# baiwenjia/ukbb_cardiac

Measured on AMD Instinct MI355X. Metric: 192x208 SAX slices/sec, higher is better.
Workload: dtype f32; 1 GPU; short-axis FCN (FCN_sa, 4 classes) inference, batch=64 synthetic 192x208 slices per GPU resident in HBM, int32 label map out (BASELINE.json configs[1]); height=192, width=208, weights=synthetic seed 1234, parallelism=batch split x1, no collectives

## Files before the change

### include/ukbb_fcn.h

```cpp
#ifndef UKBB_FCN_H
#define UKBB_FCN_H

#include <stddef.h>
#include <stdint.h>

#ifdef __cplusplus
extern "C" {
#endif

#define UKBB_FCN_ABI_VERSION 11
#define UKBB_FCN_MAX_LEVEL 8

#define UKBB_OK 0
#define UKBB_EINVAL (-1)
#define UKBB_EARCH (-2)
#define UKBB_EDEVICE (-3)
#define UKBB_ENOMEM (-4)

#define UKBB_KIND_FCN 0
#define UKBB_KIND_UNET 1
#define UKBB_KIND_UNET_LSTM 2
#define UKBB_KIND_TEMPORAL_UNET 3

typedef struct ukbb_fcn_arch {
// ... 79 lines not shown
                           int64_t st, double mu, double den, int X2, int Y2, int x_pre, int y_pre, float *d_batch, void *stream);


int ukbb_fcn_label_components(const uint8_t *d_lab, int X, int Y, int Z, int T, int n_class, int min_size, int32_t *d_work,
                              int32_t *d_n_large, void *stream);

int ukbb_fcn_label_max(const void *d_vol, int nifti_datatype, int X, int Y, int Z, int T, int64_t sx, int64_t sy, int64_t sz, int64_t st,
                       const uint8_t *d_lab, int n_class, double *d_max, void *stream);

int ukbb_fcn_label_compact(const void *d_vol, int nifti_datatype, int X, int Y, int Z, int64_t sx, int64_t sy, int64_t sz, const uint8_t *d_lab,
                           int label, void *d_out, uint64_t *n_host, void *stream);

uint64_t ukbb_fcn_gzip_labels_bound(uint64_t n_voxels, int nifti_datatype, uint64_t prefix_len);
int64_t ukbb_fcn_gzip_labels(const uint8_t *labels, uint64_t n_voxels, int nifti_datatype, const uint8_t *prefix, uint64_t prefix_len,
                             uint8_t *out, uint64_t out_cap);
#define UKBB_GZIP_FIXED 0
#define UKBB_GZIP_DYNAMIC 1
int64_t ukbb_fcn_gzip_labels_mode(const uint8_t *labels, uint64_t n_voxels, int nifti_datatype, const uint8_t *prefix, uint64_t prefix_len,
                                  uint8_t *out, uint64_t out_cap, int mode);

int64_t ukbb_fcn_gunzip(const uint8_t *src, uint64_t src_len, uint8_t *dst, uint64_t dst_cap, int verify_crc);
uint32_t ukbb_fcn_gzip_crc(uint32_t crc, const uint8_t *data, uint64_t n);


int ukbb_fcn_num_kernels(const ukbb_fcn_handle *h);
const char *ukbb_fcn_kernel_name(const ukbb_fcn_handle *h, int i);
double ukbb_fcn_kernel_macs(const ukbb_fcn_handle *h, int i);
double ukbb_fcn_kernel_mfma_macs(const ukbb_fcn_handle *h, int i);
double ukbb_fcn_kernel_mfma_macs_issued(const ukbb_fcn_handle *h, int i);

int ukbb_fcn_kernel_config(const ukbb_fcn_handle *h, int i);
const char *ukbb_fcn_conv_config_name(int id);

int ukbb_fcn_set_timing(ukbb_fcn_handle *h, int enable);
int ukbb_fcn_set_timing_kernel(ukbb_fcn_handle *h, int kernel);
int ukbb_fcn_kernel_times(ukbb_fcn_handle *h, double *sum_ms, int64_t *count, int n, int reset);

int64_t ukbb_fcn_get_activation(ukbb_fcn_handle *h, const char *name, float *dst, int64_t cap);

int ukbb_fcn_clock_probe(int device, void *stream, int spin_us, double *mhz);

int ukbb_fcn_synth_volume(uint64_t seed, size_t n, float *d_out, void *stream);

#ifdef __cplusplus
}
#endif
#endif
```

### ukbb_cardiac_amd/_lib.py

```python
import ctypes as C
import os

import numpy as np

_HERE = os.path.dirname(os.path.abspath(__file__))
LIB_PATH = os.environ.get('UKBB_FCN_LIB') or os.path.join(_HERE, 'libukbb_fcn.so')
ABI_VERSION = 11
MAX_LEVEL = 8

EXPORTS = [
    'ukbb_fcn_abi_version', 'ukbb_fcn_last_error', 'ukbb_fcn_weight_count', 'ukbb_fcn_create',
    'ukbb_fcn_destroy', 'ukbb_fcn_reserve', 'ukbb_fcn_forward', 'ukbb_fcn_forward_host',
    'ukbb_fcn_num_kernels', 'ukbb_fcn_kernel_name', 'ukbb_fcn_kernel_macs', 'ukbb_fcn_set_timing',
    'ukbb_fcn_kernel_times', 'ukbb_fcn_get_activation', 'ukbb_fcn_kernel_config', 'ukbb_fcn_conv_config_name',
    'ukbb_fcn_set_timing_kernel', 'ukbb_fcn_set_precision', 'ukbb_fcn_kernel_mfma_macs',
    'ukbb_fcn_select_kth', 'ukbb_fcn_rescale_pack', 'ukbb_fcn_unpack_labels',
    'ukbb_fcn_roi_compact', 'ukbb_fcn_pairwise_sum', 'ukbb_fcn_zscore_pack',
    'ukbb_fcn_gzip_labels_bound', 'ukbb_fcn_gzip_labels', 'ukbb_fcn_gzip_labels_mode', 'ukbb_fcn_gunzip', 'ukbb_fcn_gzip_crc',
    'ukbb_fcn_forward_seq', 'ukbb_fcn_forward_cine', 'ukbb_fcn_clock_probe', 'ukbb_fcn_kernel_mfma_macs_issued',
    'ukbb_fcn_synth_volume',
    'ukbb_fcn_select_kth_t', 'ukbb_fcn_rescale_pack_t', 'ukbb_fcn_roi_compact_t', 'ukbb_fcn_pairwise_sum_t', 'ukbb_fcn_zscore_pack_t',
    'ukbb_fcn_label_components', 'ukbb_fcn_label_max', 'ukbb_fcn_label_compact',
    'ukbb_fcn_set_scratch_budget', 'ukbb_fcn_scratch_bytes', 'ukbb_fcn_cine_scratch_bytes',
    'ukbb_fcn_cine_min_scratch_bytes', 'ukbb_fcn_cine_chunk_windows',
]


class ArchStruct(C.Structure):
    _fields_ = [('kind', C.c_int32), ('n_class', C.c_int32), ('n_level', C.c_int32),
                ('n_filter', C.c_int32 * MAX_LEVEL), ('n_block', C.c_int32 * MAX_LEVEL),
                ('same_dim', C.c_int32), ('fc', C.c_int32)]


def arch_struct(arch) -> ArchStruct:
    s = ArchStruct()
    s.kind, s.n_class, s.n_level = arch.kind, arch.n_class, arch.n_level
    for i in range(arch.n_level):
        s.n_filter[i] = arch.n_filter[i]
        s.n_block[i] = arch.n_block[i]
    s.same_dim, s.fc = arch.same_dim, arch.fc
    return s


def _load():
    if not os.path.exists(LIB_PATH):
        raise ImportError(
            'ukbb_cardiac_amd: %s is missing. Build the gfx950 HIP library first '
# ... 118 lines not shown
```

### ukbb_cardiac_amd/csrc/engine.cpp

```cpp
#include "../../include/ukbb_fcn.h"
#include "kernels.h"

#include <algorithm>
#include <cmath>
#include <cstdarg>
#include <cstdio>
#include <cstdlib>
#include <cstring>
#include <map>
#include <memory>
#include <string>
#include <vector>

using namespace ukbb;

extern "C" int ukbb_fcn_debug_poison_lds(uint32_t pattern, void *stream);
extern "C" int ukbb_fcn_debug_fence_kernel(void *stream);

namespace {

thread_local std::string g_err;

void set_err(const char *fmt, ...) {
    char buf[1024];
// ... 2024 lines not shown

double ukbb_fcn_kernel_mfma_macs(const ukbb_fcn_handle *h, int i) {
    if (!h || i < 0 || i >= (int)h->ops.size()) return 0.0;
    const Op &op = h->ops[i];
    return (op.mfma_macs_per_image >= 0 ? op.mfma_macs_per_image : op.macs_per_image) * h->last_n;
}

double ukbb_fcn_kernel_mfma_macs_issued(const ukbb_fcn_handle *h, int i) {
    if (!h || i < 0 || i >= (int)h->ops.size()) return 0.0;
    const Op &op = h->ops[i];
    if (op.padded_macs_per_image >= 0) return op.padded_macs_per_image * h->last_n;
    return ukbb_fcn_kernel_mfma_macs(h, i);
}

int ukbb_fcn_set_precision(ukbb_fcn_handle *h, int precision) {
    if (!h || (precision != UKBB_PREC_FP32 && precision != UKBB_PREC_BF16 && precision != UKBB_PREC_F32X3)) { set_err("set_precision: bad argument"); return UKBB_EINVAL; }
    if (h->arch.kind == UKBB_KIND_TEMPORAL_UNET && precision == UKBB_PREC_BF16) {
        set_err("set_precision: the Temporal-UNet's 3-D convolutions are built for fp32 only (no bf16 plan)");
        return UKBB_EARCH;
    }
    if (precision != h->precision) {
        if (hipSetDevice(h->device) != hipSuccess || hipDeviceSynchronize() != hipSuccess) { set_err("set_precision: device sync failed"); return UKBB_EDEVICE; }
        h->precision = precision;
        h->plan_h = h->plan_w = 0;
    }
    return UKBB_OK;
}

int ukbb_fcn_kernel_config(const ukbb_fcn_handle *h, int i) {
    if (!h || i < 0 || i >= (int)h->ops.size() || (h->ops[i].kind != OP_CONV && h->ops[i].kind != OP_TCONV)) return -1;
    return h->ops[i].cfg;
}

const char *ukbb_fcn_conv_config_name(int id) {
    for (int i = 0; i < num_conv_configs(); ++i)
        if (conv_config(i).id == id) return conv_config(i).name;
    return "";
}

int ukbb_fcn_set_timing(ukbb_fcn_handle *h, int enable) {
    if (!h) { set_err("set_timing: NULL handle"); return UKBB_EINVAL; }
    int rc = collect_events(h);
    if (rc) return rc;
    h->timing = enable != 0;
    h->timing_only = -1;
    return UKBB_OK;
}

int ukbb_fcn_set_timing_kernel(ukbb_fcn_handle *h, int kernel) {
    if (!h) { set_err("set_timing_kernel: NULL handle"); return UKBB_EINVAL; }
    int rc = collect_events(h);
    if (rc) return rc;
    if (kernel >= (int)h->ops.size()) { set_err("set_timing_kernel: index out of range"); return UKBB_EINVAL; }
    h->timing = true;
    h->timing_only = kernel < 0 ? -1 : kernel;
    return UKBB_OK;
}

int ukbb_fcn_kernel_times(ukbb_fcn_handle *h, double *sum_ms, int64_t *count, int n, int reset) {
    if (!h) { set_err("kernel_times: NULL handle"); return UKBB_EINVAL; }
    int rc = collect_events(h);
    if (rc) return rc;
    const int m = std::min<int>(n, (int)h->ops.size());
    for (int i = 0; i < m; ++i) {
        if (sum_ms) sum_ms[i] = h->t_sum[i];
        if (count) count[i] = h->t_cnt[i];
// ... 56 lines not shown
```

### ukbb_cardiac_amd/csrc/kernels.h

```cpp
#pragma once
#include <hip/hip_runtime.h>
#include <stdint.h>

#include "device_state.h"

namespace ukbb {

inline int current_device() { int d = 0; return hipGetDevice(&d) == hipSuccess ? d : -1; }
inline int device_cu_count() {
    static PerDeviceInt cu;
    const int d = current_device();
    return cu.get(d, [d] { hipDeviceProp_t p; return d >= 0 && hipGetDeviceProperties(&p, d) == hipSuccess ? p.multiProcessorCount : 0; }, 256);
}
inline hipError_t allow_dynamic_lds(OncePerDevice &once, const void *kernel, int bytes) {
    return (hipError_t)once.run(current_device(), [&] {
        return (int)hipFuncSetAttribute(kernel, hipFuncAttributeMaxDynamicSharedMemorySize, bytes); });
}

template <int NCLS>
__device__ __forceinline__ int softmax_argmax(const float (&lg)[NCLS], float *p) {
    int best = 0; float m = lg[0];
#pragma unroll
    for (int c = 1; c < NCLS; ++c) if (lg[c] > m) { m = lg[c]; best = c; }
    bool near = false;
// ... 120 lines not shown
    const float *x;
    const float *w_s;
    const float *b_s;
    const float *w_g;
    float *out;
    long long npix;
    int cin;
};
hipError_t launch_sqg(const SqgArgs &a, hipStream_t s);
struct SqgMultiArgs { SqgArgs lv[4]; int nb[4]; };
hipError_t launch_sqg_multi(const SqgArgs lv[4], hipStream_t s);

struct HeadArgs {
    const float *conv0;
    const float *G[4];
    const float *w_s0;
    const float *b_s0;
    const float *w_o0;
    const float *b_o0;
    const float *w_o1;
    const float *b_o1;
    const float *w_o0x3;
    const float *w_o1x3;
    const float *w_lg;
    const float *b_lg;
    float *logits;
    float *prob;
    int32_t *pred;
    int N, H, W, n_class;
    int x3;
    int diag;
};
hipError_t launch_head(const HeadArgs &a, hipStream_t s);
void pack_sq(const float *w , int cin, float *dst );
void pack_rowmap_32x64(const float *w , int ld, float *dst );
void pack_head_lg(const float *w , int n_class, float *dst );
void pack_head_x3(const float *w , int k_in , float *dst );

void tconv_as_conv2x2(const float *w, int cin, int cout, float *dst);

struct TailArgs {
    const float *in0, *in1;
    const float *wA0, *wA1;
    const float *b0, *b1;
    const float *lg_w, *lg_b;
    float *logits, *prob;
    int32_t *pred;
    int N, H, W, ncls;
    unsigned long long *stamps;
    int seg_tiles;
};
hipError_t launch_unet_tail(const TailArgs &a, hipStream_t s);
void pack_tail_weights(const float *w0 , const float *w1 , float *dst0 , float *dst1 );

struct StemArgs {
    const float *image;
    const float *wA0, *wA1;
    const float *b0, *b1;
    float *out;
    int N, H, W;
};
hipError_t launch_unet_stem(const StemArgs &a, hipStream_t s);
void pack_stem_weights(const float *w0 , float *dst0 );

struct LogitsArgs {
    const float *in;
// ... 91 lines not shown
```

### ukbb_cardiac_amd/csrc/kernels_head.hip

```cpp
#include "kernels.h"

#include <cstdio>

#include <cstdlib>
#include <cstring>
#include <type_traits>

namespace ukbb {

typedef float f32x16 __attribute__((ext_vector_type(16)));
typedef float f32x4 __attribute__((ext_vector_type(4)));

__host__ __device__ __forceinline__ constexpr int rowmap(int r, int g) {
    return (r & 3) + 8 * (r >> 2) + 4 * g;
}

typedef float f32x2 __attribute__((ext_vector_type(2)));
typedef unsigned u32x4 __attribute__((ext_vector_type(4)));
#ifdef UKBB_NO_PACKED_F32
__device__ __forceinline__ float s_fma(float a, float b, float c) { float r; asm("v_fma_f32 %0, %1, %2, %3" : "=v"(r) : "v"(a), "v"(b), "v"(c)); return r; }
__device__ __forceinline__ f32x2 pk_fma(f32x2 a, f32x2 b, f32x2 c) { return f32x2{s_fma(a[0], b[0], c[0]), s_fma(a[1], b[1], c[1])}; }
#else
__device__ __forceinline__ f32x2 pk_fma(f32x2 a, f32x2 b, f32x2 c) {
    f32x2 r; asm("v_pk_fma_f32 %0, %1, %2, %3" : "=v"(r) : "v"(a), "v"(b), "v"(c)); return r;
}
#endif
#define MFMA32(a, b, c) __builtin_amdgcn_mfma_f32_32x32x2f32((a), (b), (c), 0, 0, 0)

__device__ __forceinline__ f32x4 ldg4(const float *p) { return *reinterpret_cast<const f32x4 *>(p); }

__device__ __forceinline__ f32x16 bias_tile(const float *bias, int g) {
    f32x16 acc;
#pragma unroll
    for (int j = 0; j < 4; ++j) {
// ... 345 lines not shown
            float s = 0.f;
#pragma unroll
            for (int j = 0; j < 4; ++j) {
                const f32x4 w = ldg4(wp + 4 * j);
#pragma unroll
                for (int i = 0; i < 4; ++i) s = fmaf(w[i], Q0[4 * j + i], s);
            }
#pragma unroll
            for (int j = 0; j < 4; ++j) {
                const f32x4 w = ldg4(wp + 16 + 4 * j);
#pragma unroll
                for (int i = 0; i < 4; ++i) s = fmaf(w[i], Q1[4 * j + i], s);
            }
            const float other = __shfl_xor(s, 32);
            lg[c] = (g == 0 ? s + other : other + s) + a.b_lg[c];
        }
        if (g == 0) {
            if (a.logits) {
#pragma unroll
                for (int c = 0; c < NCLS; ++c) a.logits[q * NCLS + c] = lg[c];
            }
            float pr[NCLS];
            const int best = softmax_argmax_opt<NCLS>(lg, a.prob != nullptr, pr);
            if (a.pred) a.pred[q] = best;
            if (a.prob) {
#pragma unroll
                for (int c = 0; c < NCLS; ++c) a.prob[q * NCLS + c] = pr[c];
            }
        }
    }
}

#ifdef UKBB_DIAG
__device__ unsigned long long g_hstamps[8];
#endif
constexpr int PX_WAVE = 8 * 64 * 4;
constexpr int L_GW = 0;
constexpr int L_PX = L_GW + 2 * GPIX * GSTRIDE;
template <bool X3> struct HeadLds {
    static constexpr int WS0 = L_PX + 4 * PX_WAVE;
    static constexpr int WO0 = WS0 + 512;
    static constexpr int WO1 = WO0 + (X3 ? 3072 : 2048);
    static constexpr int BS0 = WO1 + (X3 ? 6144 : 4096);
    static constexpr int BO0 = BS0 + 32;
    static constexpr int BO1 = BO0 + 64;
    static constexpr int WLG = BO1 + 64;
    static constexpr int BLG = WLG + 384;
    static constexpr int FLOATS = BLG + 8;
};
constexpr int HEADPC_LDS_FLOATS = HeadLds<false>::FLOATS;
constexpr int HEADPC_X3_LDS_FLOATS = HeadLds<true>::FLOATS;
static_assert(HEADPC_X3_LDS_FLOATS * 4 <= 160 * 1024, "head kernel LDS");

__device__ __forceinline__ f32x4 lds4(const float *p) { return *reinterpret_cast<const f32x4 *>(p); }

template <int N, int I = 0, class F>
__device__ __forceinline__ void unroll_n(F &&f) {
    if constexpr (I < N) { f(std::integral_constant<int, I>{}); unroll_n<N, I + 1>(f); }
}

__device__ __forceinline__ f32x16 bias_tile_lds(const float *bias, int g) {
    f32x16 acc;
#pragma unroll
    for (int j = 0; j < 4; ++j) {
        const f32x4 b = lds4(bias + 8 * j + 4 * g);
#pragma unroll
        for (int i = 0; i < 4; ++i) acc[4 * j + i] = b[i];
    }
    return acc;
}

__device__ __forceinline__ void chain_32to64_lds(const float *wp, int lane, const f32x16 &X, f32x16 &D0, f32x16 &D1) {
#pragma unroll
    for (int q4 = 0; q4 < 4; ++q4) {
        const f32x4 wa = lds4(wp + ((0 * 4 + q4) * 64 + lane) * 4);
        const f32x4 wb = lds4(wp + ((1 * 4 + q4) * 64 + lane) * 4);
#pragma unroll
        for (int i = 0; i < 4; ++i) {
            D0 = MFMA32(wa[i], X[4 * q4 + i], D0);
            D1 = MFMA32(wb[i], X[4 * q4 + i], D1);
        }
    }
}

typedef __bf16 hbf16x8 __attribute__((ext_vector_type(8)));
__device__ __forceinline__ unsigned pk_bf16(float lo, float hi) {
    const __bf16 l = (__bf16)lo, h = (__bf16)hi;
    return (unsigned)__builtin_bit_cast(unsigned short, l) | ((unsigned)__builtin_bit_cast(unsigned short, h) << 16);
}
__device__ __forceinline__ void split_pair(float x0, float x1, unsigned &h, unsigned &m, unsigned &l) {
    h = pk_bf16(x0, x1);
    const float r0 = x0 - __builtin_bit_cast(float, h << 16), r1 = x1 - __builtin_bit_cast(float, h & 0xffff0000u);
    m = pk_bf16(r0, r1);
    const float q0 = r0 - __builtin_bit_cast(float, m << 16), q1 = r1 - __builtin_bit_cast(float, m & 0xffff0000u);
    l = pk_bf16(q0, q1);
}
__device__ __forceinline__ f32x16 mfma_b16(const u32x4 &a, const u32x4 &b, const f32x16 &c) {
    return __builtin_amdgcn_mfma_f32_32x32x16_bf16(__builtin_bit_cast(hbf16x8, a), __builtin_bit_cast(hbf16x8, b), c, 0, 0, 0);
}

__host__ __device__ constexpr int sep_pb(int l) { return ((1 << l) - 1) >> 1; }
__host__ __device__ constexpr int sep_row0(int r0, int l) { return (r0 + sep_pb(l)) >> l; }
__host__ __device__ constexpr bool sep_row_used(int r0, int l, int k) {
    const int f = 1 << l, i = sep_row0(r0, l) + k;
    bool used = false;
    for (int t = 0; t < 4; ++t) {
        const int y = r0 + t + sep_pb(l);
        if ((y >> l) + 1 == i || ((y >> l) == i && (y & (f - 1)) != f - 1)) used = true;
    }
    return used;
}

template <int NCLS, bool X3 = false, bool DG = false>
__global__ __launch_bounds__(768) void fcn_head_pc_kernel(const HeadArgs a) {
    extern __shared__ __attribute__((aligned(16))) float lds[];
    using LM = HeadLds<X3>;
    constexpr int L_WS0 = LM::WS0, L_WO0 = LM::WO0, L_WO1 = LM::WO1, L_BS0 = LM::BS0, L_BO0 = LM::BO0, L_BO1 = LM::BO1, L_WLG = LM::WLG, L_BLG = LM::BLG;
    float *gw = lds + L_GW;
    float *px = lds + L_PX;
    const int tiles_x = a.W / HT, tiles_y = a.H / HT;
    const int ntiles = a.N * tiles_y * tiles_x;
    const int my_tiles = (ntiles - (int)blockIdx.x + (int)gridDim.x - 1) / (int)gridDim.x;
    const int nstages = 2 * my_tiles;
    const bool producer = __builtin_amdgcn_readfirstlane(threadIdx.x) >= 256;
    const int lane = threadIdx.x & 63, p = lane & 31, g = lane >> 5;

    {
        const int t = threadIdx.x;
        auto copy = [&](int dst, const float *src, int nfloat) {
            for (int i = t; i < nfloat; i += 768) lds[dst + i] = src[i];
        };
        copy(L_WS0, a.w_s0, 512);
        if constexpr (X3) { copy(L_WO0, a.w_o0x3, 3072); copy(L_WO1, a.w_o1x3, 6144); }
        else              { copy(L_WO0, a.w_o0, 2048);   copy(L_WO1, a.w_o1, 4096); }
        copy(L_BS0, a.b_s0, 32);  copy(L_BO0, a.b_o0, 64);   copy(L_BO1, a.b_o1, 64);
        copy(L_WLG, a.w_lg, 2 * NCLS * 32); copy(L_BLG, a.b_lg, NCLS);
    }

    if (producer) {
        const int tid = threadIdx.x - 256, pw = (tid >> 6) & 3, half = tid >> 8;
        constexpr int NIT = 7;
        u32x4 gv[NIT];
        const int sp32 = tid >> 4, c4 = tid & 15;
#ifndef UKBB_HEAD_RECOMPUTE_WINDOW_CONSTS
#define UKBB_HEAD_RECOMPUTE_WINDOW_CONSTS 0
#endif
// ... 164 lines not shown
        };
        if (my_tiles > 0) { g_load(0); g_store(0); }
        if (my_tiles > 1) { g_load(1); g_store(1); }
        __syncthreads();
        auto stage = [&](auto parc, auto bufc, auto rgc, int s) {
            constexpr int PAR = decltype(parc)::value, BUF = decltype(bufc)::value;
            if constexpr (DG) {
                gather(parc, bufc);
                hand_over();
            } else {
                gather_sep(parc, bufc, rgc);
                hand_over_sep(rgc);
            }
            __syncthreads();
            __syncthreads();
            if constexpr (PAR == 1) {
                const int k = s >> 1;
                if (k + 2 < my_tiles) { g_load(k + 2); g_store(BUF); }
            }
        };
        constexpr std::integral_constant<int, 0> I0{};
        constexpr std::integral_constant<int, 1> I1{};
        auto run = [&](auto rgc) {
#pragma unroll 1
            for (int s = 0; s < nstages; s += 4) {
                stage(I0, I0, rgc, s);
                stage(I1, I0, rgc, s + 1);
                if (s + 2 < nstages) { stage(I0, I1, rgc, s + 2); stage(I1, I1, rgc, s + 3); }
            }
        };
        if constexpr (DG) run(I0);
        else if (__builtin_amdgcn_readfirstlane(tid) < 256) run(I0);
        else run(I1);
    } else {
        const int wave = threadIdx.x >> 6;
        const float *w_s0 = lds + L_WS0, *w_o0 = lds + L_WO0, *w_o1 = lds + L_WO1, *w_lg = lds + L_WLG;
        auto pixel_of = [&](int s) -> size_t {
            int bid = blockIdx.x + (s >> 1) * gridDim.x;
            const int tx = bid % tiles_x; bid /= tiles_x;
            const int ty = bid % tiles_y;
            const int n = bid / tiles_y;
            const int blk = DG ? wave * 2 + (s & 1) : 4 * (s & 1) + wave;
            const int y = ty * HT + 2 * blk + (p >> 4), x = tx * HT + (p & 15);
            return ((size_t)n * a.H + y) * a.W + x;
        };
        f32x4 xv0 = {0.f, 0.f, 0.f, 0.f}, xv1 = xv0;
        if (nstages > 0) {
            const size_t q0 = pixel_of(0);
            xv0 = ldg4(a.conv0 + q0 * 16 + 4 * g);
            xv1 = ldg4(a.conv0 + q0 * 16 + 8 + 4 * g);
        }
        __syncthreads();
#ifdef UKBB_DIAG
        unsigned long long hs_a = 0, hs_r = 0, hs_b = 0, hs_t0 = __builtin_amdgcn_s_memtime();
#define UKBB_HS(var, prev) { asm volatile("s_waitcnt lgkmcnt(0)" ::: "memory"); const unsigned long long t_ = __builtin_amdgcn_s_memtime(); var += t_ - prev; prev = t_; }
#else
#define UKBB_HS(var, prev)
#endif
#pragma unroll 1
        for (int s = 0; s < nstages; ++s) {
            const size_t q = pixel_of(s);
            const f32x4 x0 = xv0, x1 = xv1;
#ifdef UKBB_DIAG
            unsigned long long hs_p = __builtin_amdgcn_s_memtime();
#endif
            __syncthreads();
            UKBB_HS(hs_a, hs_p)
            f32x16 P0, P1;
            {
                const float *src = px + wave * PX_WAVE + lane * 4;
#pragma unroll
                for (int j = 0; j < 4; ++j) {
                    const f32x4 v0 = lds4(src + j * 256);
                    const f32x4 v1 = lds4(src + (4 + j) * 256);
#pragma unroll
                    for (int i = 0; i < 4; ++i) { P0[4 * j + i] = v0[i]; P1[4 * j + i] = v1[i]; }
                }
            }
            UKBB_HS(hs_r, hs_p)
            __syncthreads();
            UKBB_HS(hs_b, hs_p)
            if (s + 1 < nstages) {
                const size_t qn = pixel_of(s + 1);
                xv0 = ldg4(a.conv0 + qn * 16 + 4 * g);
                xv1 = ldg4(a.conv0 + qn * 16 + 8 + 4 * g);
            }
            f32x16 S = bias_tile_lds(lds + L_BS0, g);
            {
                const f32x4 wv0 = lds4(w_s0 + lane * 4), wv1 = lds4(w_s0 + (64 + lane) * 4);
#pragma unroll
                for (int i = 0; i < 4; ++i) S = MFMA32(wv0[i], x0[i], S);
#pragma unroll
                for (int i = 0; i < 4; ++i) S = MFMA32(wv1[i], x1[i], S);
            }
            relu16(S);
#ifdef UKBB_DIAG
            if (a.diag & 2) { relu16(P0); relu16(P1); if (a.pred) a.pred[q] = (int)P0[0]; continue; }
#endif
            if constexpr (X3) {
                u32x4 sh[2], sm[2], sl[2];
#pragma unroll
                for (int kc = 0; kc < 2; ++kc)
#pragma unroll
                    for (int d = 0; d < 4; ++d) {
                        unsigned th, tm, tl;
                        split_pair(S[8 * kc + 2 * d], S[8 * kc + 2 * d + 1], th, tm, tl);
                        sh[kc][d] = th; sm[kc][d] = tm; sl[kc][d] = tl;
                    }
                const float *wx0 = lds + L_WO0 + lane * 4;
                auto A0 = [&](int t, int cb, int kc) { return __builtin_bit_cast(u32x4, lds4(wx0 + ((t * 2 + cb) * 2 + kc) * 256)); };
#pragma unroll
                for (int kc = 0; kc < 2; ++kc) {
                    const u32x4 ah0 = A0(0, 0, kc), ah1 = A0(0, 1, kc), am0 = A0(1, 0, kc), am1 = A0(1, 1, kc), al0 = A0(2, 0, kc), al1 = A0(2, 1, kc);
                    P0 = mfma_b16(al0, sh[kc], P0); P1 = mfma_b16(al1, sh[kc], P1);
                    P0 = mfma_b16(ah0, sl[kc], P0); P1 = mfma_b16(ah1, sl[kc], P1);
                    P0 = mfma_b16(am0, sm[kc], P0); P1 = mfma_b16(am1, sm[kc], P1);
                    P0 = mfma_b16(am0, sh[kc], P0); P1 = mfma_b16(am1, sh[kc], P1);
                    P0 = mfma_b16(ah0, sm[kc], P0); P1 = mfma_b16(ah1, sm[kc], P1);
                    P0 = mfma_b16(ah0, sh[kc], P0); P1 = mfma_b16(ah1, sh[kc], P1);
                }
            } else {
                chain_32to64_lds(w_o0, lane, S, P0, P1);
            }
            relu16(P0);
            relu16(P1);
            f32x16 Q0 = bias_tile_lds(lds + L_BO1, g), Q1 = bias_tile_lds(lds + L_BO1 + 32, g);
            if constexpr (X3) {
                u32x4 bh[4], bm[4], bl[4];
                auto split = [&](auto kcc) {
                    constexpr int kc = decltype(kcc)::value;
#pragma unroll
                    for (int d = 0; d < 4; ++d) {
                        constexpr int r0 = 8 * (kc & 1);
                        const float x0 = kc < 2 ? P0[r0 + 2 * d] : P1[r0 + 2 * d], x1 = kc < 2 ? P0[r0 + 2 * d + 1] : P1[r0 + 2 * d + 1];
                        unsigned th, tm, tl;
                        split_pair(x0, x1, th, tm, tl);
                        bh[kc][d] = th; bm[kc][d] = tm; bl[kc][d] = tl;
                    }
                };
                const float *wx = lds + L_WO1 + lane * 4;
                auto A = [&](int t, int cb, int kc) { return __builtin_bit_cast(u32x4, lds4(wx + ((t * 2 + cb) * 4 + kc) * 256)); };
                split(std::integral_constant<int, 0>{});
                unroll_n<4>([&](auto kcc) {
                    constexpr int kc = decltype(kcc)::value;
                    const u32x4 ah0 = A(0, 0, kc), ah1 = A(0, 1, kc), am0 = A(1, 0, kc), am1 = A(1, 1, kc), al0 = A(2, 0, kc), al1 = A(2, 1, kc);
                    if constexpr (kc < 3) split(std::integral_constant<int, kc + 1>{});
                    Q0 = mfma_b16(al0, bh[kc], Q0); Q1 = mfma_b16(al1, bh[kc], Q1);
                    Q0 = mfma_b16(ah0, bl[kc], Q0); Q1 = mfma_b16(ah1, bl[kc], Q1);
                    Q0 = mfma_b16(am0, bm[kc], Q0); Q1 = mfma_b16(am1, bm[kc], Q1);
                    Q0 = mfma_b16(am0, bh[kc], Q0); Q1 = mfma_b16(am1, bh[kc], Q1);
                    Q0 = mfma_b16(ah0, bm[kc], Q0); Q1 = mfma_b16(ah1, bm[kc], Q1);
                    Q0 = mfma_b16(ah0, bh[kc], Q0); Q1 = mfma_b16(ah1, bh[kc], Q1);
                    if constexpr (kc < 3) {
#pragma unroll
                        for (int i = 0; i < 12; ++i) {
                            __builtin_amdgcn_sched_group_barrier(0x008, 1, 0);
                            __builtin_amdgcn_sched_group_barrier(0x002, 5, 0);
                        }
                    }
                });
            } else {
                chain_32to64_lds(w_o1, lane, P0, Q0, Q1);
                chain_32to64_lds(w_o1 + 2 * 4 * 64 * 4, lane, P1, Q0, Q1);
            }
            relu16(Q0);
            relu16(Q1);
#ifdef UKBB_DIAG
            if (a.diag & 4) { if (a.pred) a.pred[q] = (int)(Q0[0] + Q1[0]); continue; }
#endif
            float lg[NCLS];
#pragma unroll
            for (int c = 0; c < NCLS; ++c) {
                const float *wp = w_lg + (g * NCLS + c) * 32;
                f32x2 acc2 = {0.f, 0.f};
#pragma unroll
                for (int j = 0; j < 4; ++j) {
                    const f32x4 w = lds4(wp + 4 * j);
                    acc2 = pk_fma(f32x2{w[0], w[1]}, f32x2{Q0[4 * j], Q0[4 * j + 1]}, acc2);
                    acc2 = pk_fma(f32x2{w[2], w[3]}, f32x2{Q0[4 * j + 2], Q0[4 * j + 3]}, acc2);
                }
#pragma unroll
                for (int j = 0; j < 4; ++j) {
                    const f32x4 w = lds4(wp + 16 + 4 * j);
                    acc2 = pk_fma(f32x2{w[0], w[1]}, f32x2{Q1[4 * j], Q1[4 * j + 1]}, acc2);
                    acc2 = pk_fma(f32x2{w[2], w[3]}, f32x2{Q1[4 * j + 2], Q1[4 * j + 3]}, acc2);
                }
                const float acc = acc2[0] + acc2[1];
                const float other = __shfl_xor(acc, 32);
                lg[c] = (g == 0 ? acc + other : other + acc) + lds[L_BLG + c];
            }
            if (g == 0) {
                if (a.logits) {
#pragma unroll
                    for (int c = 0; c < NCLS; ++c) a.logits[q * NCLS + c] = lg[c];
                }
                float pr[NCLS];
                const int best = softmax_argmax_opt<NCLS>(lg, a.prob != nullptr, pr);
                if (a.pred) a.pred[q] = best;
                if (a.prob) {
#pragma unroll
                    for (int c = 0; c < NCLS; ++c) a.prob[q * NCLS + c] = pr[c];
                }
            }
        }
#ifdef UKBB_DIAG
        if (lane == 0 && (a.diag & 64)) {
            atomicAdd(g_hstamps + 0, hs_a); atomicAdd(g_hstamps + 1, hs_r); atomicAdd(g_hstamps + 2, hs_b);
            atomicAdd(g_hstamps + 3, __builtin_amdgcn_s_memtime() - hs_t0); atomicAdd(g_hstamps + 4, (unsigned long long)nstages);
        }
#endif
    }
}

static hipError_t launch_head_pc(const HeadArgs &a, hipStream_t s) {
    const int n_cu = device_cu_count();
    const int ntiles = a.N * (a.H / HT) * (a.W / HT);
    dim3 grid((unsigned)(ntiles < n_cu ? ntiles : n_cu)), block(768);
    static const bool x3_env = [] { const char *e = getenv("UKBB_HEAD_X3"); return e && atoi(e) != 0; }();
    static const bool dg = [] { const char *e = getenv("UKBB_HEAD_DIRECT_GATHER"); return e && atoi(e) != 0; }();
    if ((a.x3 || x3_env) && a.w_o1x3 && a.w_o0x3) {
        const size_t ldsx = HEADPC_X3_LDS_FLOATS * sizeof(float);
#define UKBB_HEADX3_CASE(NC)                                                                          \
    case NC: {                                                                                       \
        auto k = dg ? fcn_head_pc_kernel<NC, true, true> : fcn_head_pc_kernel<NC, true, false>;      \
        static OncePerDevice lds_ok;                                                                 \
        {                                                                                            \
            hipError_t e = allow_dynamic_lds(lds_ok, reinterpret_cast<const void *>(k), (int)ldsx);    \
            if (e != hipSuccess) return e;                                                           \
        }                                                                                            \
        hipLaunchKernelGGL(k, grid, block, ldsx, s, a);                                              \
        break;                                                                                       \
    }
        switch (a.n_class) {
            UKBB_HEADX3_CASE(2) UKBB_HEADX3_CASE(3) UKBB_HEADX3_CASE(4) UKBB_HEADX3_CASE(5) UKBB_HEADX3_CASE(6)
            default: return hipErrorInvalidValue;
        }
        return hipGetLastError();
    }
    const size_t lds = HEADPC_LDS_FLOATS * sizeof(float);
#define UKBB_HEADPC_CASE(NC)                                                                          \
    case NC: {                                                                                       \
        auto k = dg ? fcn_head_pc_kernel<NC, false, true> : fcn_head_pc_kernel<NC, false, false>;    \
        static OncePerDevice lds_ok;                                                                 \
        {                                                                                            \
            hipError_t e = allow_dynamic_lds(lds_ok, reinterpret_cast<const void *>(k), (int)lds);    \
            if (e != hipSuccess) return e;                                                           \
        }                                                                                            \
        hipLaunchKernelGGL(k, grid, block, lds, s, a);                                               \
        break;                                                                                       \
    }
    switch (a.n_class) {
        UKBB_HEADPC_CASE(2) UKBB_HEADPC_CASE(3) UKBB_HEADPC_CASE(4) UKBB_HEADPC_CASE(5) UKBB_HEADPC_CASE(6)
        default: return hipErrorInvalidValue;
    }
    return hipGetLastError();
}

template <int OCC>
static hipError_t launch_head_occ(const HeadArgs &a, hipStream_t s) {
    dim3 grid((unsigned)(a.N * (a.H / HT) * (a.W / HT))), block(256);
    const size_t lds = HEAD_LDS_FLOATS * sizeof(float);
    switch (a.n_class) {
        case 2: hipLaunchKernelGGL((fcn_head_kernel<2, OCC>), grid, block, lds, s, a); break;
        case 3: hipLaunchKernelGGL((fcn_head_kernel<3, OCC>), grid, block, lds, s, a); break;
        case 4: hipLaunchKernelGGL((fcn_head_kernel<4, OCC>), grid, block, lds, s, a); break;
        case 5: hipLaunchKernelGGL((fcn_head_kernel<5, OCC>), grid, block, lds, s, a); break;
        case 6: hipLaunchKernelGGL((fcn_head_kernel<6, OCC>), grid, block, lds, s, a); break;
        default: return hipErrorInvalidValue;
    }
    return hipGetLastError();
}

hipError_t launch_head(const HeadArgs &a_in, hipStream_t s) {
    HeadArgs a = a_in;
#ifdef UKBB_DIAG
    { const char *e = getenv("UKBB_HEAD_DIAG"); a.diag = e ? atoi(e) : 0; }
#endif
    if ((a.H % HT) || (a.W % HT)) return hipErrorInvalidValue;
    static const int use_pc = [] { const char *e = getenv("UKBB_HEAD_PC"); return e ? atoi(e) : 1; }();
#ifdef UKBB_DIAG
    if (use_pc && getenv("UKBB_HEAD_STAMPS")) {
        static int shots = 0;
        unsigned long long z[8] = {0};
        a.diag |= 64;
        (void)hipMemcpyToSymbol(HIP_SYMBOL(g_hstamps), z, 64);
        const hipError_t e = launch_head_pc(a, s);
        (void)hipStreamSynchronize(s);
        if (++shots == 6) {
            unsigned long long h[8];
            (void)hipMemcpyFromSymbol(h, HIP_SYMBOL(g_hstamps), 64);
            const double st = (double)h[4];
            if (st > 0) fprintf(stderr, "[head stamps] per MFMA wave and stage (32-pixel block): wait at barrier A (hand-off) %.0f, read of the handed tile %.0f, wait at barrier B %.0f, "
                                        "MFMA chain + own vector work %.0f; total %.0f cycles\n", h[0] / st, h[1] / st, h[2] / st, (h[3] - h[0] - h[1] - h[2]) / st, h[3] / st);
        }
        return e;
    }
#endif
    if (use_pc) return launch_head_pc(a, s);
    const HeadArgs &b = a;
    static const int occ = [] { const char *e = getenv("UKBB_HEAD_OCC"); return e ? atoi(e) : 3; }();
    if (occ == 2) return launch_head_occ<2>(b, s);
    if (occ == 4) return launch_head_occ<4>(b, s);
    return launch_head_occ<3>(b, s);
}

void pack_sq(const float *w, int cin, float *dst) {
    for (int j = 0; j < cin / 8; ++j)
        for (int lane = 0; lane < 64; ++lane)
            for (int i = 0; i < 4; ++i)
                dst[(j * 64 + lane) * 4 + i] = w[(8 * j + 4 * (lane >> 5) + i) * 32 + (lane & 31)];
}

void pack_rowmap_32x64(const float *w, int ld, float *dst) {
    for (int cb = 0; cb < 2; ++cb)
        for (int q4 = 0; q4 < 4; ++q4)
            for (int lane = 0; lane < 64; ++lane)
                for (int i = 0; i < 4; ++i) {
                    const int g = lane >> 5, m = lane & 31;
                    dst[(((cb * 4 + q4) * 64 + lane) * 4) + i] = w[rowmap(4 * q4 + i, g) * ld + cb * 32 + m];
                }
}

static inline unsigned short host_bf16_rne(float f) {
    unsigned u; memcpy(&u, &f, 4);
    u += 0x7fffu + ((u >> 16) & 1u);
    return (unsigned short)(u >> 16);
// ... 100 lines not shown
```

Measured before the change: 54270 slices/s.

## Defer head logits tail into next stage's MFMA chain in producer-consumer head kernel

Adds a new default consumer path for the FCN head kernel. The second half of the logits dot product, the cross-lane reduction, the softmax/argmax and the stores for one 32-pixel block are deferred and interleaved into the MFMA chains of the next stage, at fixed MFMA slots set with sched_barriers. The aim is to hide the serial vector tail behind matrix work and raise MFMA utilisation. In exchange it keeps more live registers and uses fragile hand-scheduled code; the old inline tail stays available through an environment variable.

```diff
diff --git a/include/ukbb_fcn.h b/include/ukbb_fcn.h
--- a/include/ukbb_fcn.h
+++ b/include/ukbb_fcn.h
@@ -135,6 +135,8 @@
 int ukbb_fcn_kernel_config(const ukbb_fcn_handle *h, int i);
 const char *ukbb_fcn_conv_config_name(int id);
 
+int ukbb_fcn_head_tail_form(void);
+
 int ukbb_fcn_set_timing(ukbb_fcn_handle *h, int enable);
 int ukbb_fcn_set_timing_kernel(ukbb_fcn_handle *h, int kernel);
 int ukbb_fcn_kernel_times(ukbb_fcn_handle *h, double *sum_ms, int64_t *count, int n, int reset);
diff --git a/ukbb_cardiac_amd/_lib.py b/ukbb_cardiac_amd/_lib.py
--- a/ukbb_cardiac_amd/_lib.py
+++ b/ukbb_cardiac_amd/_lib.py
@@ -13,6 +13,7 @@
     'ukbb_fcn_destroy', 'ukbb_fcn_reserve', 'ukbb_fcn_forward', 'ukbb_fcn_forward_host',
     'ukbb_fcn_num_kernels', 'ukbb_fcn_kernel_name', 'ukbb_fcn_kernel_macs', 'ukbb_fcn_set_timing',
     'ukbb_fcn_kernel_times', 'ukbb_fcn_get_activation', 'ukbb_fcn_kernel_config', 'ukbb_fcn_conv_config_name',
+    'ukbb_fcn_head_tail_form',
     'ukbb_fcn_set_timing_kernel', 'ukbb_fcn_set_precision', 'ukbb_fcn_kernel_mfma_macs',
     'ukbb_fcn_select_kth', 'ukbb_fcn_rescale_pack', 'ukbb_fcn_unpack_labels',
     'ukbb_fcn_roi_compact', 'ukbb_fcn_pairwise_sum', 'ukbb_fcn_zscore_pack',
diff --git a/ukbb_cardiac_amd/csrc/engine.cpp b/ukbb_cardiac_amd/csrc/engine.cpp
--- a/ukbb_cardiac_amd/csrc/engine.cpp
+++ b/ukbb_cardiac_amd/csrc/engine.cpp
@@ -2080,6 +2080,8 @@
     return h->ops[i].cfg;
 }
 
+int ukbb_fcn_head_tail_form(void) { return head_tail_form(); }
+
 const char *ukbb_fcn_conv_config_name(int id) {
     for (int i = 0; i < num_conv_configs(); ++i)
         if (conv_config(i).id == id) return conv_config(i).name;
diff --git a/ukbb_cardiac_amd/csrc/kernels.h b/ukbb_cardiac_amd/csrc/kernels.h
--- a/ukbb_cardiac_amd/csrc/kernels.h
+++ b/ukbb_cardiac_amd/csrc/kernels.h
@@ -176,6 +176,7 @@
     int diag;
 };
 hipError_t launch_head(const HeadArgs &a, hipStream_t s);
+int head_tail_form();
 void pack_sq(const float *w , int cin, float *dst );
 void pack_rowmap_32x64(const float *w , int ld, float *dst );
 void pack_head_lg(const float *w , int n_class, float *dst );
diff --git a/ukbb_cardiac_amd/csrc/kernels_head.hip b/ukbb_cardiac_amd/csrc/kernels_head.hip
--- a/ukbb_cardiac_amd/csrc/kernels_head.hip
+++ b/ukbb_cardiac_amd/csrc/kernels_head.hip
@@ -1,5 +1,6 @@
 #include "kernels.h"
 
+#include <atomic>
 #include <cstdio>
 
 #include <cstdlib>
@@ -411,7 +412,7 @@
 }
 
 #ifdef UKBB_DIAG
-__device__ unsigned long long g_hstamps[8];
+__device__ unsigned long long g_hstamps[16];
 #endif
 constexpr int PX_WAVE = 8 * 64 * 4;
 constexpr int L_GW = 0;
@@ -432,6 +433,10 @@
 static_assert(HEADPC_X3_LDS_FLOATS * 4 <= 160 * 1024, "head kernel LDS");
 
 __device__ __forceinline__ f32x4 lds4(const float *p) { return *reinterpret_cast<const f32x4 *>(p); }
+typedef const __attribute__((address_space(3))) float lds_cf;
+typedef const __attribute__((address_space(3))) f32x4 lds_cf4;
+__device__ __forceinline__ lds_cf *lds_opaque(const float *p) { lds_cf *q = (lds_cf *)p; asm volatile("" : "+v"(q)); return q; }
+__device__ __forceinline__ f32x4 lds4(lds_cf *p) { return *(lds_cf4 *)p; }
 
 template <int N, int I = 0, class F>
 __device__ __forceinline__ void unroll_n(F &&f) {
@@ -490,7 +495,225 @@
     return used;
 }
 
-template <int NCLS, bool X3 = false, bool DG = false>
+__host__ __device__ constexpr int fin_slot(int k) { return k < 3 ? 1 + 3 * k : 7 + 4 * (k - 2); }
+__host__ __device__ constexpr int fin_step_at(int m) {
+    for (int k = 0; k < 7; ++k) if (fin_slot(k) == m) return k;
+    return -1;
+}
+static_assert(fin_slot(2) == 7 && fin_slot(6) == 23, "tail steps end well inside out0's 32 MFMAs");
+
+#ifdef UKBB_DIAG
+#define UKBB_HS(var, prev) { __builtin_amdgcn_sched_barrier(0); asm volatile("s_waitcnt lgkmcnt(0)" ::: "memory"); const unsigned long long t_ = __builtin_amdgcn_s_memtime(); var += t_ - prev; prev = t_; __builtin_amdgcn_sched_barrier(0); }
+#else
+#define UKBB_HS(var, prev)
+#endif
+
+template <int NCLS>
+__device__ __forceinline__ void head_consumer_deferred(const HeadArgs &a, float *lds, int nstages, int tiles_x, int tiles_y) {
+    using LM = HeadLds<false>;
+    constexpr int L_WS0 = LM::WS0, L_WO0 = LM::WO0, L_WO1 = LM::WO1, L_BS0 = LM::BS0, L_BO1 = LM::BO1, L_WLG = LM::WLG, L_BLG = LM::BLG;
+    const float *px = lds + L_PX;
+    const int lane = threadIdx.x & 63, p = lane & 31, g = lane >> 5, wave = threadIdx.x >> 6;
+    auto pixel_of = [&](int s) -> size_t {
+        int bid = blockIdx.x + (s >> 1) * gridDim.x;
+        const int tx = bid % tiles_x; bid /= tiles_x;
+        const int ty = bid % tiles_y;
+        const int n = bid / tiles_y;
+        const int blk = 4 * (s & 1) + wave;
+        const int y = ty * HT + 2 * blk + (p >> 4), x = tx * HT + (p & 15);
+        return ((size_t)n * a.H + y) * a.W + x;
+    };
+    f32x4 xv0 = {0.f, 0.f, 0.f, 0.f}, xv1 = xv0;
+    size_t qnext = 0;
+    if (nstages > 0) {
+        qnext = pixel_of(0);
+        xv0 = ldg4(a.conv0 + qnext * 16 + 4 * g);
+        xv1 = ldg4(a.conv0 + qnext * 16 + 8 + 4 * g);
+    }
+    __syncthreads();
+#ifdef UKBB_DIAG
+    unsigned long long hs_a = 0, hs_r = 0, hs_b = 0, hs_j[4] = {0, 0, 0, 0}, hs_t0 = __builtin_amdgcn_s_memtime();
+#endif
+    lds_cf *const wbase = lds_opaque(lds + L_WS0 + lane * 4);
+    lds_cf *const bbase = lds_opaque(lds + L_BS0 + 4 * g);
+    lds_cf *const lbase = lds_opaque(lds + L_WLG + g * NCLS * 32);
+    auto bias_tile_at = [&](int off) {
+        f32x16 acc;
+#pragma unroll
+        for (int j = 0; j < 4; ++j) {
+            const f32x4 b = lds4(bbase + off + 8 * j);
+#pragma unroll
+            for (int i = 0; i < 4; ++i) acc[4 * j + i] = b[i];
+        }
+        return acc;
+    };
+    f32x16 Qd;
+#pragma unroll
+    for (int r = 0; r < 16; ++r) Qd[r] = 0.f;
+    f32x2 accd[NCLS];
+    f32x4 wl[NCLS];
+    float hsum[NCLS], hoth[NCLS], hbias[NCLS], lgd[NCLS];
+#pragma unroll
+    for (int c = 0; c < NCLS; ++c) accd[c] = f32x2{0.f, 0.f};
+    size_t qd = 0;
+    auto relu_n = [&](f32x16 &Q, auto r0c, auto nc) {
+#pragma unroll
+        for (int r = 0; r < decltype(nc)::value; ++r) Q[decltype(r0c)::value + r] = relu1(Q[decltype(r0c)::value + r]);
+    };
+    auto lg_load = [&](int j, int half) {
+#pragma unroll
+        for (int c = 0; c < NCLS; ++c) wl[c] = lds4(lbase + c * 32 + 16 * half + 4 * j);
+    };
+    auto half_step = [&](auto kc, auto halfc, f32x16 &Q, f32x2 (&acc)[NCLS]) {
+        constexpr int k = decltype(kc)::value, half = decltype(halfc)::value;
+        if constexpr (k == 0) { lg_load(0, half); relu_n(Q, std::integral_constant<int, 0>{}, std::integral_constant<int, 8>{}); }
+        else if constexpr (k == 1) relu_n(Q, std::integral_constant<int, 8>{}, std::integral_constant<int, 8>{});
+        else if constexpr (k <= 5) {
+            constexpr int j = k - 2;
+#pragma unroll
+            for (int c = 0; c < NCLS; ++c) acc[c] = pk_fma(f32x2{wl[c][0], wl[c][1]}, f32x2{Q[4 * j], Q[4 * j + 1]}, acc[c]);
+#pragma unroll
+            for (int c = 0; c < NCLS; ++c) acc[c] = pk_fma(f32x2{wl[c][2], wl[c][3]}, f32x2{Q[4 * j + 2], Q[4 * j + 3]}, acc[c]);
+            if constexpr (j < 3) lg_load(j + 1, half);
+        }
+    };
+    auto fin = [&](auto kc) {
+        constexpr int k = decltype(kc)::value;
+        if constexpr (k <= 5) half_step(kc, std::integral_constant<int, 1>{}, Qd, accd);
+        else if constexpr (k == 6) {
+#pragma unroll
+            for (int c = 0; c < NCLS; ++c) { hsum[c] = accd[c][0] + accd[c][1]; hbias[c] = lds[L_BLG + c]; }
+#pragma unroll
+            for (int c = 0; c < NCLS; ++c) hoth[c] = __shfl_xor(hsum[c], 32);
+        } else {
+#pragma unroll
+            for (int c = 0; c < NCLS; ++c) lgd[c] = (g == 0 ? hsum[c] + hoth[c] : hoth[c] + hsum[c]) + hbias[c];
+        }
+    };
+    auto store_tail = [&](size_t qq) {
+        if (g == 0) {
+            if (a.logits) {
+#pragma unroll
+                for (int c = 0; c < NCLS; ++c) a.logits[qq * NCLS + c] = lgd[c];
+            }
+            float pr[NCLS];
+            const int best = softmax_argmax_opt<NCLS>(lgd, a.prob != nullptr, pr);
+            if (a.pred) a.pred[qq] = best;
+            if (a.prob) {
+#pragma unroll
+                for (int c = 0; c < NCLS; ++c) a.prob[qq * NCLS + c] = pr[c];
+            }
+        }
+    };
+#pragma unroll 1
+    for (int s = 0; s < nstages; ++s) {
+        const size_t q = qnext;
+        const f32x4 x0 = xv0, x1 = xv1;
+#ifdef UKBB_DIAG
+        unsigned long long hs_p = __builtin_amdgcn_s_memtime();
+#endif
+        __syncthreads();
+        UKBB_HS(hs_a, hs_p)
+        f32x16 P0, P1;
+        {
+            const float *src = px + wave * PX_WAVE + lane * 4;
+#pragma unroll
+            for (int j = 0; j < 4; ++j) {
+                const f32x4 v0 = lds4(src + j * 256);
+                const f32x4 v1 = lds4(src + (4 + j) * 256);
+#pragma unroll
+                for (int i = 0; i < 4; ++i) { P0[4 * j + i] = v0[i]; P1[4 * j + i] = v1[i]; }
+            }
+        }
+        UKBB_HS(hs_r, hs_p)
+        __syncthreads();
+        UKBB_HS(hs_b, hs_p)
+        if (s + 1 < nstages) {
+            qnext = pixel_of(s + 1);
+            xv0 = ldg4(a.conv0 + qnext * 16 + 4 * g);
+            xv1 = ldg4(a.conv0 + qnext * 16 + 8 + 4 * g);
+        }
+        f32x16 S = bias_tile_at(0);
+        auto at_slot = [&](auto mc, auto &&mfma) {
+            constexpr int k = fin_step_at(decltype(mc)::value);
+            if constexpr (k >= 0) __builtin_amdgcn_sched_barrier(0);
+            mfma();
+            if constexpr (k >= 0) { fin(std::integral_constant<int, k>{}); __builtin_amdgcn_sched_barrier(0); }
+        };
+        constexpr int WO0 = L_WO0 - L_WS0, WO1 = L_WO1 - L_WS0;
+        f32x4 oa = lds4(wbase + WO0), ob = lds4(wbase + WO0 + 4 * 256);
+        {
+            const f32x4 wv0 = lds4(wbase), wv1 = lds4(wbase + 256);
+            unroll_n<8>([&](auto mc) {
+                constexpr int m = decltype(mc)::value;
+                at_slot(mc, [&] { S = MFMA32(m < 4 ? wv0[m & 3] : wv1[m & 3], m < 4 ? x0[m & 3] : x1[m & 3], S); });
+            });
+        }
+        relu16(S);
+        UKBB_HS(hs_j[0], hs_p)
+        unroll_n<4>([&](auto qc) {
+            constexpr int q4 = decltype(qc)::value;
+            f32x4 na = oa, nb = ob;
+            if constexpr (q4 < 3) { na = lds4(wbase + WO0 + (q4 + 1) * 256); nb = lds4(wbase + WO0 + (4 + q4 + 1) * 256); }
+            unroll_n<4>([&](auto ic) {
+                constexpr int i = decltype(ic)::value, m = 8 + 8 * q4 + 2 * i;
+                at_slot(std::integral_constant<int, m>{}, [&] { P0 = MFMA32(oa[i], S[4 * q4 + i], P0); });
+                at_slot(std::integral_constant<int, m + 1>{}, [&] { P1 = MFMA32(ob[i], S[4 * q4 + i], P1); });
+            });
+            oa = na; ob = nb;
+        });
+        f32x16 Q0 = bias_tile_at(L_BO1 - L_BS0), Q1;
+        auto wf = [&](int G) {
+            return lds4(wbase + WO1 + (((G & 4) ? 2 * 4 * 64 : 0) + ((G >> 3) * 4 + (G & 3)) * 64) * 4);
+        };
+        f32x4 wq = wf(0);
+        fin(std::integral_constant<int, 7>{});
+        if (s > 0) store_tail(qd);
+        relu16(P0);
+        UKBB_HS(hs_j[1], hs_p)
+        f32x2 acc[NCLS];
+#pragma unroll
+        for (int c = 0; c < NCLS; ++c) acc[c] = f32x2{0.f, 0.f};
+        unroll_n<16>([&](auto Gc) {
+            constexpr int G = decltype(Gc)::value, k = G & 7;
+            f32x4 wn = wq;
+            if constexpr (G < 15) wn = wf(G + 1);
+            if constexpr (G == 6) Q1 = bias_tile_at(L_BO1 - L_BS0 + 32);
+            unroll_n<4>([&](auto ic) {
+                constexpr int i = decltype(ic)::value, slot = 4 * G + i;
+                constexpr bool relu_p1 = slot >= 1 && slot <= 4, head = slot >= 33 && slot <= 53 && (slot - 33) % 4 == 0;
+                const float xb = k < 4 ? P0[4 * (k & 3) + i] : P1[4 * (k & 3) + i];
+                if constexpr (relu_p1 || head) __builtin_amdgcn_sched_barrier(0);
+                if constexpr (G < 8) Q0 = MFMA32(wq[i], xb, Q0);
+                else Q1 = MFMA32(wq[i], xb, Q1);
+                if constexpr (head) asm volatile("" : "+v"(Q1));
+                if constexpr (relu_p1) relu_n(P1, std::integral_constant<int, 4 * (slot - 1)>{}, std::integral_constant<int, 4>{});
+                if constexpr (head) half_step(std::integral_constant<int, (slot - 33) / 4>{}, std::integral_constant<int, 0>{}, Q0, acc);
+                if constexpr (relu_p1 || head) __builtin_amdgcn_sched_barrier(0);
+            });
+            wq = wn;
+        });
+        UKBB_HS(hs_j[2], hs_p)
+        Qd = Q1;
+#pragma unroll
+        for (int c = 0; c < NCLS; ++c) accd[c] = acc[c];
+        qd = q;
+    }
+    if (nstages > 0) {
+        unroll_n<8>([&](auto kc) { fin(kc); });
+        store_tail(qd);
+    }
+#ifdef UKBB_DIAG
+    if (lane == 0 && (a.diag & 64)) {
+        atomicAdd(g_hstamps + 0, hs_a); atomicAdd(g_hstamps + 1, hs_r); atomicAdd(g_hstamps + 2, hs_b);
+        atomicAdd(g_hstamps + 3, __builtin_amdgcn_s_memtime() - hs_t0); atomicAdd(g_hstamps + 4, (unsigned long long)nstages);
+#pragma unroll
+        for (int j = 0; j < 4; ++j) atomicAdd(g_hstamps + 5 + j, hs_j[j]);
+    }
+#endif
+}
+
+template <int NCLS, bool X3 = false, bool DG = false, bool IT = true>
 __global__ __launch_bounds__(768) void fcn_head_pc_kernel(const HeadArgs a) {
     extern __shared__ __attribute__((aligned(16))) float lds[];
     using LM = HeadLds<X3>;
@@ -721,6 +944,8 @@
         if constexpr (DG) run(I0);
         else if (__builtin_amdgcn_readfirstlane(tid) < 256) run(I0);
         else run(I1);
+    } else if constexpr (!X3 && !DG && !IT) {
+        head_consumer_deferred<NCLS>(a, lds, nstages, tiles_x, tiles_y);
     } else {
         const int wave = threadIdx.x >> 6;
         const float *w_s0 = lds + L_WS0, *w_o0 = lds + L_WO0, *w_o1 = lds + L_WO1, *w_lg = lds + L_WLG;
@@ -741,10 +966,7 @@
         }
         __syncthreads();
 #ifdef UKBB_DIAG
-        unsigned long long hs_a = 0, hs_r = 0, hs_b = 0, hs_t0 = __builtin_amdgcn_s_memtime();
-#define UKBB_HS(var, prev) { asm volatile("s_waitcnt lgkmcnt(0)" ::: "memory"); const unsigned long long t_ = __builtin_amdgcn_s_memtime(); var += t_ - prev; prev = t_; }
-#else
-#define UKBB_HS(var, prev)
+        unsigned long long hs_a = 0, hs_r = 0, hs_b = 0, hs_j[4] = {0, 0, 0, 0}, hs_t0 = __builtin_amdgcn_s_memtime();
 #endif
 #pragma unroll 1
         for (int s = 0; s < nstages; ++s) {
@@ -783,6 +1005,7 @@
                 for (int i = 0; i < 4; ++i) S = MFMA32(wv1[i], x1[i], S);
             }
             relu16(S);
+            UKBB_HS(hs_j[0], hs_p)
 #ifdef UKBB_DIAG
             if (a.diag & 2) { relu16(P0); relu16(P1); if (a.pred) a.pred[q] = (int)P0[0]; continue; }
 #endif
@@ -813,6 +1036,7 @@
             }
             relu16(P0);
             relu16(P1);
+            UKBB_HS(hs_j[1], hs_p)
             f32x16 Q0 = bias_tile_lds(lds + L_BO1, g), Q1 = bias_tile_lds(lds + L_BO1 + 32, g);
             if constexpr (X3) {
                 u32x4 bh[4], bm[4], bl[4];
@@ -854,6 +1078,7 @@
             }
             relu16(Q0);
             relu16(Q1);
+            UKBB_HS(hs_j[2], hs_p)
 #ifdef UKBB_DIAG
             if (a.diag & 4) { if (a.pred) a.pred[q] = (int)(Q0[0] + Q1[0]); continue; }
 #endif
@@ -891,58 +1116,63 @@
                     for (int c = 0; c < NCLS; ++c) a.prob[q * NCLS + c] = pr[c];
                 }
             }
+            UKBB_HS(hs_j[3], hs_p)
         }
 #ifdef UKBB_DIAG
         if (lane == 0 && (a.diag & 64)) {
             atomicAdd(g_hstamps + 0, hs_a); atomicAdd(g_hstamps + 1, hs_r); atomicAdd(g_hstamps + 2, hs_b);
             atomicAdd(g_hstamps + 3, __builtin_amdgcn_s_memtime() - hs_t0); atomicAdd(g_hstamps + 4, (unsigned long long)nstages);
-        }
-#endif
-    }
+#pragma unroll
+            for (int j = 0; j < 4; ++j) atomicAdd(g_hstamps + 5 + j, hs_j[j]);
+        }
+#endif
+    }
+}
+
+template <int NC, bool X3, bool DG, bool IT>
+static hipError_t launch_head_pc_inst(const HeadArgs &a, dim3 grid, size_t lds_bytes, hipStream_t s) {
+    static OncePerDevice lds_ok;
+    const hipError_t e = allow_dynamic_lds(lds_ok, reinterpret_cast<const void *>(fcn_head_pc_kernel<NC, X3, DG, IT>), (int)lds_bytes);
+    if (e != hipSuccess) return e;
+    hipLaunchKernelGGL((fcn_head_pc_kernel<NC, X3, DG, IT>), grid, dim3(768), lds_bytes, s, a);
+    return hipGetLastError();
+}
+
+static std::atomic<int> g_head_tail_form{-1};
+int head_tail_form() { return g_head_tail_form.load(std::memory_order_relaxed); }
+
+template <int NC>
+static hipError_t launch_head_pc_nc(const HeadArgs &a, dim3 grid, hipStream_t s) {
+    static const bool x3_env = [] { const char *e = getenv("UKBB_HEAD_X3"); return e && atoi(e) != 0; }();
+    static const bool dg = [] { const char *e = getenv("UKBB_HEAD_DIRECT_GATHER"); return e && atoi(e) != 0; }();
+    static const bool inline_tail = [] { const char *e = getenv("UKBB_HEAD_INLINE_TAIL"); return e && atoi(e) != 0; }();
+    if ((a.x3 || x3_env) && a.w_o1x3 && a.w_o0x3) {
+        const size_t ldsx = HEADPC_X3_LDS_FLOATS * sizeof(float);
+        g_head_tail_form.store(1, std::memory_order_relaxed);
+        return dg ? launch_head_pc_inst<NC, true, true, true>(a, grid, ldsx, s) : launch_head_pc_inst<NC, true, false, true>(a, grid, ldsx, s);
+    }
+    const size_t lds = HEADPC_LDS_FLOATS * sizeof(float);
+    bool it = inline_tail;
+#ifdef UKBB_DIAG
+    if (a.diag & 6) it = true;
+#endif
+    g_head_tail_form.store(dg || it ? 1 : 0, std::memory_order_relaxed);
+    if (dg) return launch_head_pc_inst<NC, false, true, true>(a, grid, lds, s);
+    return it ? launch_head_pc_inst<NC, false, false, true>(a, grid, lds, s) : launch_head_pc_inst<NC, false, false, false>(a, grid, lds, s);
 }
 
 static hipError_t launch_head_pc(const HeadArgs &a, hipStream_t s) {
     const int n_cu = device_cu_count();
     const int ntiles = a.N * (a.H / HT) * (a.W / HT);
-    dim3 grid((unsigned)(ntiles < n_cu ? ntiles : n_cu)), block(768);
-    static const bool x3_env = [] { const char *e = getenv("UKBB_HEAD_X3"); return e && atoi(e) != 0; }();
-    static const bool dg = [] { const char *e = getenv("UKBB_HEAD_DIRECT_GATHER"); return e && atoi(e) != 0; }();
-    if ((a.x3 || x3_env) && a.w_o1x3 && a.w_o0x3) {
-        const size_t ldsx = HEADPC_X3_LDS_FLOATS * sizeof(float);
-#define UKBB_HEADX3_CASE(NC)                                                                          \
-    case NC: {                                                                                       \
-        auto k = dg ? fcn_head_pc_kernel<NC, true, true> : fcn_head_pc_kernel<NC, true, false>;      \
-        static OncePerDevice lds_ok;                                                                 \
-        {                                                                                            \
-            hipError_t e = allow_dynamic_lds(lds_ok, reinterpret_cast<const void *>(k), (int)ldsx);    \
-            if (e != hipSuccess) return e;                                                           \
-        }                                                                                            \
-        hipLaunchKernelGGL(k, grid, block, ldsx, s, a);                                              \
-        break;                                                                                       \
-    }
-        switch (a.n_class) {
-            UKBB_HEADX3_CASE(2) UKBB_HEADX3_CASE(3) UKBB_HEADX3_CASE(4) UKBB_HEADX3_CASE(5) UKBB_HEADX3_CASE(6)
-            default: return hipErrorInvalidValue;
-        }
-        return hipGetLastError();
-    }
-    const size_t lds = HEADPC_LDS_FLOATS * sizeof(float);
-#define UKBB_HEADPC_CASE(NC)                                                                          \
-    case NC: {                                                                                       \
-        auto k = dg ? fcn_head_pc_kernel<NC, false, true> : fcn_head_pc_kernel<NC, false, false>;    \
-        static OncePerDevice lds_ok;                                                                 \
-        {                                                                                            \
-            hipError_t e = allow_dynamic_lds(lds_ok, reinterpret_cast<const void *>(k), (int)lds);    \
-            if (e != hipSuccess) return e;                                                           \
-        }                                                                                            \
-        hipLaunchKernelGGL(k, grid, block, lds, s, a);                                               \
-        break;                                                                                       \
-    }
+    dim3 grid((unsigned)(ntiles < n_cu ? ntiles : n_cu));
     switch (a.n_class) {
-        UKBB_HEADPC_CASE(2) UKBB_HEADPC_CASE(3) UKBB_HEADPC_CASE(4) UKBB_HEADPC_CASE(5) UKBB_HEADPC_CASE(6)
+        case 2: return launch_head_pc_nc<2>(a, grid, s);
+        case 3: return launch_head_pc_nc<3>(a, grid, s);
+        case 4: return launch_head_pc_nc<4>(a, grid, s);
+        case 5: return launch_head_pc_nc<5>(a, grid, s);
+        case 6: return launch_head_pc_nc<6>(a, grid, s);
         default: return hipErrorInvalidValue;
     }
-    return hipGetLastError();
 }
 
 template <int OCC>
@@ -970,17 +1200,20 @@
 #ifdef UKBB_DIAG
     if (use_pc && getenv("UKBB_HEAD_STAMPS")) {
         static int shots = 0;
-        unsigned long long z[8] = {0};
+        unsigned long long z[16] = {0};
         a.diag |= 64;
-        (void)hipMemcpyToSymbol(HIP_SYMBOL(g_hstamps), z, 64);
+        (void)hipMemcpyToSymbol(HIP_SYMBOL(g_hstamps), z, sizeof(z));
         const hipError_t e = launch_head_pc(a, s);
         (void)hipStreamSynchronize(s);
         if (++shots == 6) {
-            unsigned long long h[8];
-            (void)hipMemcpyFromSymbol(h, HIP_SYMBOL(g_hstamps), 64);
+            unsigned long long h[16];
+            (void)hipMemcpyFromSymbol(h, HIP_SYMBOL(g_hstamps), sizeof(h));
             const double st = (double)h[4];
             if (st > 0) fprintf(stderr, "[head stamps] per MFMA wave and stage (32-pixel block): wait at barrier A (hand-off) %.0f, read of the handed tile %.0f, wait at barrier B %.0f, "
                                         "MFMA chain + own vector work %.0f; total %.0f cycles\n", h[0] / st, h[1] / st, h[2] / st, (h[3] - h[0] - h[1] - h[2]) / st, h[3] / st);
+            if (st > 0) fprintf(stderr, "[head stamps] of it: same_dim0 + ReLU %.0f, out0 + ReLU %.0f, out1 + ReLU %.0f, logits to store %.0f; outside the stamps "
+                                        "(prologue, prefetch issue, flush) %.0f\n", h[5] / st, h[6] / st, h[7] / st, h[8] / st,
+                                (h[3] - h[0] - h[1] - h[2] - h[5] - h[6] - h[7] - h[8]) / st);
         }
         return e;
     }
```

Result: faster. 55660 slices/s (median of 6 runs) (+2.6%).
